# olibridge01/TeXOCR

Measured on AMD Instinct MI355X. Metric: images/sec (OCRModel.generate, greedy, max_len=256, 224x672 px), higher is better.
Workload: dtype bf16; 1 GPU; BASELINE configs[1]: config.yml dims (256-d/8h/4L enc + 4L dec, patch 16, PatchEmbedding C=3), batch 64/GPU, 224x672, greedy max_len=256; global_batch=64, parallelism=dp1 (images sharded, single process, no collective)

## Files before the change

### texocr_amd/csrc/engine.hip

```cpp
#include "../../include/texocr.h"

#include <hip/hip_runtime.h>
#include <hip/hip_ext.h>

#include <algorithm>
#include <array>
#include <cmath>
#include <cstdio>
#include <cstdlib>
#include <chrono>
#include <cstring>
#include <map>
#include <memory>
#include <string>
#include <type_traits>
#include <vector>

namespace txo {
static thread_local std::string g_err;
static int fail(int code, const std::string& msg) { g_err = msg; return code; }
}
#define HIP_TRY(expr)                                                                                   \
    do {                                                                                                \
        hipError_t _e = (expr);                                                                         \
// ... 722 lines not shown
            conv<TB>(s, act[2], b.c2, act[3], B, hc, wc, b.mid, b.mid, 3, b.stride, ri);
            group_norm<true, false>(s, (const TB*)act[3], (const TB*)nullptr, act[3], b.n2, B, ho * wo, b.mid, ro, wo);
            conv<TB>(s, act[3], b.c3, act[2], B, ho, wo, b.mid, b.cout, 1, 1, ro);
            group_norm<true, true>(s, (const TB*)act[2], res, act[0], b.n3, B, ho * wo, b.cout, ro, wo);
            cur = act[0]; hc = ho; wc = wo; mul /= b.stride;
        }
        if (hc != H / 16 || wc != W / 16) return fail(TXO_E_INVALID, "backbone output grid does not match H/16 x W/16");
        *feat = cur;
        HIP_TRY(hipGetLastError());
        return 0;
    }

    int check_image_size(const std::string& who, const char* is, int H, int W, int Hc, int Wc) {
        if (H <= 0 || W <= 0 || H % 16 || W % 16) return fail(TXO_E_INVALID, who + " height/width must be positive multiples of 16");
        if (H > Hc || W > Wc) return fail(TXO_E_INVALID, who + is + "larger than the container");
        if (H > cfg.canvas_h || W > cfg.canvas_w) return fail(TXO_E_INVALID, who + is + "larger than the position-embedding canvas");
        return 0;
    }
    int fixed_batch(int B, int C, int H, int W, ImageBatch* ib) {
        if (!ready) return fail(TXO_E_STATE, "weights not finalized");
        if (C != cfg.in_channels) return fail(TXO_E_INVALID, "image channel count does not match in_channels");
        if (int r = check_image_size("image", " ", H, W, H, W)) return r;
        const int N = 1 + (H / 16) * (W / 16);
        if (B < 1 || B > Bmax) return fail(TXO_E_INVALID, "batch exceeds engine max_batch");
        if (N > Nmax) return fail(TXO_E_INVALID, "token count exceeds engine max_tokens");
        *ib = ImageBatch{B, C, H, W, N};
        return 0;
    }
    int encode(const float* img, int B, int C, int H, int W, float* enc_out, hipStream_t s) override {
        ImageBatch ib;
        if (int r = fixed_batch(B, C, H, W, &ib)) return r;
        return encode_batch(ib, img, enc_out, s);
    }
    int encode_batch(const ImageBatch& ib, const float* img, float* enc_out, hipStream_t s) {
        hipEvent_t e0 = nullptr, e1 = nullptr;
        if (prof) { e0 = pool.next(); e1 = pool.next(); (void)hipEventRecord(e0, s); }
        const int bc = enc_chunk_images(ib.B);
        for (int b0 = 0; b0 < ib.B; b0 += bc) {
            const int nb = std::min(bc, ib.B - b0);
            if (int r = encode_images(ib.chunk(b0, nb), img + b0 * ib.pixels(), enc_out + (size_t)b0 * ib.N * D, s)) return r;
        }
        if (prof) { (void)hipEventRecord(e1, s); ev_enc.push_back({e0, e1}); }
        HIP_TRY(hipGetLastError());
        return 0;
    }
    int enc_chunk_images(int B) const { return knobs.enc_chunk_env > 0 ? std::min(B, knobs.enc_chunk_env) : B; }
    void launch_patch_embed(hipStream_t s, const ImageBatch& ib, const float* img) {
        const int hw = ib.N - 1, w = ib.W / 16, G = cfg.canvas_w / 16;
        const int* rhw = rag_hw + 2 * ib.first;
        auto go = [&](auto load, auto epi) { launch_gemm_big<T>(s, load, patch_w, ib.B * hw, D, ib.C * 256, epi); };
        if (ib.ragged) go(LoadPatchRagged<T>{img, rhw, ib.C, ib.H, ib.W, hw}, EpiPatchRagged{ex, patch_b, pos, rhw, D, hw, G});
        else go(LoadPatch<T>{img, ib.C, ib.H, ib.W, hw, w}, EpiPatch{ex, patch_b, pos, D, hw, w, G});
    }
    const int* ragged_tokens(const ImageBatch& ib) const { return ib.ragged ? rag_ntok + ib.first : nullptr; }
    void launch_enc_attn_f32(hipStream_t s, const ImageBatch& ib, dim3 grid, size_t hs) {
        auto kern = ib.ragged ? enc_attn_kernel<T, true> : enc_attn_kernel<T, false>;
        hipLaunchKernelGGL(kern, grid, dim3(256), 0, s, eqkv, eqkv + hs, eqkv + 2 * hs, eao, ib.N, cfg.enc_heads, ib.B * cfg.enc_heads, ragged_tokens(ib));
    }
    void launch_enc_attn_bf16(hipStream_t s, const ImageBatch& ib, dim3 grid, size_t hs, int rev) {
        const bf16* qb = reinterpret_cast<const bf16*>(eqkv);
        auto kern = ib.ragged ? enc_attn_bf16_v2_kernel<T, true> : enc_attn_bf16_v2_kernel<T, false>;
        hipLaunchKernelGGL(kern, grid, dim3(256), 0, s, qb, qb + hs, qb + 2 * hs, eao, ib.N, cfg.enc_heads, ib.B * cfg.enc_heads, rev, ragged_tokens(ib));
    }
    int encode_images(const ImageBatch& ib, const float* img, float* enc_out, hipStream_t s) {
        const int B = ib.B, H = ib.H, W = ib.W, N = ib.N, hw = N - 1, w = W / 16;
        const int M = B * N, G = cfg.canvas_w / 16;

        hipLaunchKernelGGL(cls_rows_kernel, dim3((B * D + 255) / 256), dim3(256), 0, s, ex, cls, pos, B, N, D);
        if (!hybrid) launch_patch_embed(s, ib, img);
        else if (ib.ragged) {
            const int* rhw = rag_hw + 2 * ib.first;
            const int Hb = rag_box[0], Wb = rag_box[1], hwC = (Hb / 16) * (Wb / 16);
            const size_t n4 = (size_t)M * (D / 4);
            hipLaunchKernelGGL(zero_pad_rows_kernel, dim3((unsigned)((n4 + 255) / 256)), dim3(256), 0, s, ex, ragged_tokens(ib), B, N, D / 4);
            const EpiTokensRagged epi{ex, patch_b, pos, rhw, D, hwC, Wb / 16, N, G};
            if (bk_fp32) {
                const float* feat = nullptr;
                if (int r = backbone<float>(bk32, img, B, Hb, Wb, &feat, s, rhw, H, W)) return r;
                bk_gemm(s, LoadPlain<float>{feat, 1024}, (const float*)bk32.proj_w, B * hwC, D, 1024, epi);
            } else {
                const T* feat = nullptr;
                if (int r = backbone<T>(bk, img, B, Hb, Wb, &feat, s, rhw, H, W)) return r;
                gemm_plain(s, feat, patch_w, B * hwC, D, 1024, epi);
            }
        } else {
            if (bk_fp32) {
                const float* feat = nullptr;
                if (int r = backbone<float>(bk32, img, B, H, W, &feat, s)) return r;
                bk_gemm(s, LoadPlain<float>{feat, 1024}, (const float*)bk32.proj_w, B * hw, D, 1024, EpiTokens{ex, patch_b, pos, D, hw, w, G});
            } else {
                const T* feat = nullptr;
                if (int r = backbone<T>(bk, img, B, H, W, &feat, s)) return r;
                gemm_plain(s, feat, patch_w, B * hw, D, 1024, EpiTokens{ex, patch_b, pos, D, hw, w, G});
            }
        }
        const size_t hs = (size_t)M * Ie;
        bool down = false;
        auto dir = [&]() -> int { if (sizeof(T) != 2) return 0; const bool d = down; down = !down; return d ? 1 : 0; };
        for (int l = 0; l < cfg.enc_layers; ++l) {
            const ResidLN res_x{ey, estats, enc_gb, D}, res_first{ex, nullptr, nullptr, D};
            if (l == 0) launch_ln<0, T>(s, ex, nullptr, ez, enc_g, enc_b, M, dir());
            else launch_ln<3, T>(s, ey, estats, ez, enc_g, enc_b, M, dir());
            const dim3 agrid = ea_grid((N + EA_QBLK - 1) / EA_QBLK, B * cfg.enc_heads);
            if constexpr (sizeof(T) == 4) {
                gemm_plain(s, ez, enc_attn[l].wqkv, M, 3 * Ie, D, EpiHeads<float>{eqkv, hs, Ie, cfg.enc_heads, N});
                launch_enc_attn_f32(s, ib, agrid, hs);
            } else {
                gemm_plain(s, ez, enc_attn[l].wqkv, M, 3 * Ie, D, EpiHeads<bf16>{reinterpret_cast<bf16*>(eqkv), hs, Ie, cfg.enc_heads, N}, dir());
                launch_enc_attn_bf16(s, ib, agrid, hs, dir());
            }
            gemm_plain(s, eao, enc_attn[l].wo, M, 2 * D, Ie,
                               EpiGluRes<sizeof(T) == 2>{ey, l == 0 ? res_first : res_x, enc_attn[l].bo}, dir());
            launch_ln<3, T>(s, ey, estats, ez, enc_g, enc_b, M, dir());
            gemm_plain(s, ez, enc_mlp[l].w1, M, 2 * Fe, D, EpiGeglu<T>{ehid, enc_mlp[l].b1, Fe}, dir());
            gemm_plain(s, ehid, enc_mlp[l].w2, M, D, Fe, EpiBiasRes{ey, res_x, enc_mlp[l].b2}, dir());
        }
        launch_ln<2, float>(s, ey, nullptr, enc_out, encn_g, encn_b, M, dir());
        if (ib.ragged) {
            const size_t n4 = (size_t)M * (D / 4);
            hipLaunchKernelGGL(zero_pad_rows_kernel, dim3((unsigned)((n4 + 255) / 256)), dim3(256), 0, s, enc_out, ragged_tokens(ib), B, N, D / 4);
        }
        return 0;
    }

    int upload_i32(const int32_t* src, int* dst0, int n0, int* dst1, int n1, hipStream_t s) {
        if (rag_ev_pending) { HIP_TRY(hipEventSynchronize(rag_ev)); rag_ev_pending = false; }
        memcpy(rag_host, src, sizeof(int32_t) * (n0 + n1));
        HIP_TRY(hipMemcpyAsync(dst0, rag_host, sizeof(int32_t) * n0, hipMemcpyHostToDevice, s));
        if (n1 > 0) HIP_TRY(hipMemcpyAsync(dst1, rag_host + n0, sizeof(int32_t) * n1, hipMemcpyHostToDevice, s));
        HIP_TRY(hipEventRecord(rag_ev, s));
        rag_ev_pending = true;
        return 0;
    }
    struct Staging { void* dev; const void* host; size_t bytes; };
    template <typename Fill> int ingest_stage(int B, Staging st, hipStream_t s, bool pending, Fill fill) {
        if (B > Bmax) return fail(TXO_E_INVALID, "ingest: batch exceeds engine max_batch (the descriptor staging holds max_batch images)");
        if (ing_ev_pending) { HIP_TRY(hipEventSynchronize(ing_ev)); ing_ev_pending = false; }
        if (int r = fill()) return r;
        HIP_TRY(hipMemcpyAsync(st.dev, st.host, st.bytes, hipMemcpyHostToDevice, s));
        if (pending) { HIP_TRY(hipEventRecord(ing_ev, s)); ing_ev_pending = true; }
        return 0;
    }
    template <typename... P> int ingest_launch(void (*kern)(P...), dim3 grid, dim3 blk, hipStream_t s, typename std::common_type<P>::type... args) {
        if (!prof) { hipLaunchKernelGGL(kern, grid, blk, 0, s, args...); return 0; }
        hipEvent_t e0 = pool.next(), e1 = pool.next();
        if (!e0 || !e1) return fail(TXO_E_HIP, "hipEventCreate failed");
        hipExtLaunchKernelGGL(kern, grid, blk, 0, s, e0, e1, 0, args...);
        ev_ingest.push_back({e0, e1});
        return 0;
    }
// ... 133 lines not shown
    int check_length(int max_len, bool ragged) {
        if (max_len < 1) return fail(TXO_E_INVALID, "max_len must be >= 1");
        if (max_len <= Tmax) return 0;
        if (ragged && !rag_fwd)
            return fail(TXO_E_INVALID, "ragged batches: max_len exceeds the decoder's max_length (the sliding window of a ragged batch needs txo_set_ragged_forward(e, 1))");
        if (V % 8 == 0 && (size_t)Tmax <= (size_t)Bmax * Nmax) return 0;
        return fail(TXO_E_INVALID, ragged ? "ragged batches: max_len exceeds the decoder's max_length and the sliding window's multi-position forward needs a "
                                            "vocabulary size that is a multiple of 8 and max_length <= max_batch * max_tokens"
                                          : "max_len exceeds the decoder's max_length and the sliding window's multi-position forward needs a vocabulary "
                                            "size that is a multiple of 8 and max_length <= max_batch * max_tokens (use decoder.generate's stepwise loop)");
    }
    int check_prefix(const DecodeReq& q, int* m, int* M) {
        const int B = q.src.B, P = q.P;
        if (q.max_len < 1) return fail(TXO_E_INVALID, "prefix decode: max_len must be >= 1");
        if (B < 1 || B > Bmax) return fail(TXO_E_INVALID, "prefix decode: batch exceeds engine max_batch");
        if (P < 1) return fail(TXO_E_INVALID, "prefix decode: the prefix needs at least one column");
        *m = *M = P;
        if (q.prefix_len) {
            *M = 1;
            for (int b = 0; b < B; ++b) {
                if (q.prefix_len[b] < 1 || q.prefix_len[b] > P)
                    return fail(TXO_E_INVALID, "prefix decode: prefix_len[" + std::to_string(b) + "] must be in [1, P]");
                *m = std::min(*m, (int)q.prefix_len[b]); *M = std::max(*M, (int)q.prefix_len[b]);
            }
        }
        if ((long long)*M - 1 + q.max_len > Tmax)
            return fail(TXO_E_INVALID, "prefix decode: the longest prefix - 1 + max_len exceeds the decoder's max_length (a prompted decode does not slide the window)");
        if ((size_t)(*m - 1) > (size_t)Bmax * Nmax)
            return fail(TXO_E_INVALID, "prefix decode: the shortest prefix does not fit the multi-position pass's workspace (max_batch * max_tokens rows)");
        return 0;
    }

    int decode_begin(const float* enc, int B, int N, int eos, hipStream_t s) override { return begin_session(enc, B, N, eos, s, true); }
    int begin_session(const float* enc, int B, int N, int eos, hipStream_t s, bool project_kv, KeyCounts kc = {}, int beams = 1) {
        if (!ready) return fail(TXO_E_STATE, "weights not finalized");
        if (B < 1 || B > Bmax) return fail(TXO_E_INVALID, "batch exceeds engine max_batch");
        if (N < 1 || N > Nmax) return fail(TXO_E_INVALID, "token count exceeds engine max_tokens");
        if (kc.host) { if (int r = upload_i32(kc.host, slens, B, nullptr, 0, s)) return r; }
        if (kc.dev) HIP_TRY(hipMemcpyAsync(slens, kc.dev, sizeof(int) * B, hipMemcpyDeviceToDevice, s));
        {
            const size_t n4 = (size_t)B * N * D / 4;
            hipLaunchKernelGGL((cast_rows_kernel<T>), dim3((n4 + 255) / 256), dim3(256), 0, s, enc, enc_t, n4);
        }
        ses = Session{B * beams, N, B, true, kc.dev || kc.host, project_kv && latent_ok && knobs.lat_mode == 1};
        if (!ses.latent && project_kv) ensure_ckv(s);
        lanes.split(ses.rows, 1, s);
        reset_lanes(s, eos);
        HIP_TRY(hipGetLastError());
        return 0;
    }
    void choose_form(bool row_stop, hipStream_t s) {
        ses.latent = !ses.ragged && latent_ok && (knobs.lat_mode == 1 || (knobs.lat_mode < 0 && auto_latent(ses.rows)));
        ses.row_stop = row_stop;
        ses.lat_self = ses.latent && lat_self_ok() && !row_stop;
        if (!ses.latent) ensure_ckv(s);
    }

    void ensure_ckv(hipStream_t s) {
        if (ses.ckv_valid) return;
        const int M = ses.images * ses.keys;
        gemm_plain(s, enc_t, wckv, M, cfg.dec_layers * 2 * Id, D, EpiHeads<T>{ckv, (size_t)M * Id, Id, cfg.dec_heads, ses.keys});
        ses.ckv_valid = true;
    }

    int abandon_lanes(hipStream_t s, int rc) { stamps.slot = -1; return lanes.abandon(s, ses.images, rc); }
    void reset_lanes(hipStream_t s, int eos, int start_m = 0) {
        for (int i = 0; i < lanes.n; ++i) {
            const LaneSet::Lane& ln = lanes[i];
            const int n = ln.nb > Tmax ? ln.nb : Tmax;
            if (start_m > 0) {
                (void)hipMemsetAsync(st + i, 0, sizeof(StepState), s);
                hipLaunchKernelGGL(prefix_start_kernel, dim3((n + 255) / 256), dim3(256), 0, s, st + i, cur_tok + ln.b0, eos_seen + ln.b0,
                                   done_flag + (size_t)i * Tmax, ln.nb, Tmax, eos, ftab + (size_t)ln.b0 * Tmax, Tmax, flen + ln.b0, start_m);
// ... 559 lines not shown
        }
        if (last_logits) {
            DecGemmArgs<T> f{};
            f.rows = B; f.D = D; f.inner = Id; f.heads = heads; f.tmax = Tmax; f.t_host = t - 1; f.t_ptr = &st[0].t;
            f.N = V; f.K = D; f.W = wlog; f.bias = blog; f.logits = last_logits; f.y = dy; f.gamma = decn_g; f.beta = decn_b;
            if (int r = launch_dec_gemm<PRO_LNF, EPI_LOGITS>(s, f)) return r;
        }
        HIP_TRY(hipGetLastError());
        return 0;
    }

    static constexpr int PERSIST_MAX_BF16_GREEDY = 128;
    bool persist_usable(int B) const {
        if (sample_mode && V > 64 * SR_PER) return false;
        if (prof || prof_cross || g_dbg || knobs.run.stamps || knobs.run.graph >= 0 || knobs.run.lanes > 0) return false;
        if (ses.ragged) return false;
        if (ses.forced) return false;
        if (ses.ruled) return false;
        if (cfg.dec_exp != 4 || cfg.dec_layers > PS_MAXLD) return false;
        const bool exists = (D == 256 && cfg.dec_heads == 8) || (D == 768 && cfg.dec_heads == 12 && sizeof(T) == 2);
        if (!exists) return false;
        if (latent_ok && knobs.lat_mode == 1) return false;
        if (knobs.run.persist >= 0) return knobs.run.persist != 0;
        if (persist_cooldown > 0) return false;
        if (D != 256) return false;
        if (sizeof(T) == 2 && B > PERSIST_MAX_BF16_GREEDY) return false;
        return B <= 256;
    }
    template <int D_, int H_>
    int launch_persist(const PersistArgs<T>& pa, hipStream_t s) {
        const size_t lds = persist_lds_bytes<T, D_, H_>();
        auto kern = pa.logp_out ? (sample_mode ? decode_persist_kernel<T, D_, H_, true, true> : decode_persist_kernel<T, D_, H_, false, true>)
                                : (sample_mode ? decode_persist_kernel<T, D_, H_, true, false> : decode_persist_kernel<T, D_, H_, false, false>);
        if (hipFuncSetAttribute(reinterpret_cast<const void*>(kern), hipFuncAttributeMaxDynamicSharedMemorySize, (int)lds) != hipSuccess) {
            (void)hipGetLastError();
            return fail(TXO_E_STATE, "persistent decode: the device refused the launch's dynamic LDS size");
        }
        if (prof_persist && pool.used + 2 <= pool.ev.size()) {
            hipEvent_t e0 = pool.next(), e1 = pool.next();
            hipExtLaunchKernelGGL(kern, dim3(PS_TEAMS * PS_TEAM_BLOCKS), dim3(PS_THREADS), lds, s, e0, e1, 0, pa);
            ev_persist.push_back({e0, e1});
        } else {
            hipLaunchKernelGGL(kern, dim3(PS_TEAMS * PS_TEAM_BLOCKS), dim3(PS_THREADS), lds, s, pa);
        }
        return 0;
    }
    int generate_persist(const Decode& d, int n_pos, int* n_steps, bool* broke, hipStream_t s) {
        const int B = d.src.B, N = d.src.N, eos = d.q.eos, max_len = n_pos;
        PersistArgs<T> pa{};
        pa.B = B; pa.N = N; pa.V = V; pa.Ld = cfg.dec_layers; pa.Tmax = Tmax; pa.max_len = max_len; pa.eos = eos; pa.bos = cfg.bos;
        for (int l = 0; l < cfg.dec_layers; ++l) {
            PersistLayer<T>& L = pa.L[l];
            L.wqkv = dec_self[l].wqkv; L.wo_s = dec_self[l].wo; L.bo_s = dec_self[l].bo;
            L.wq_c = dec_cross[l].wq; L.wo_c = dec_cross[l].wo; L.bo_c = dec_cross[l].bo;
            L.w1 = dec_mlp[l].w1; L.b1 = dec_mlp[l].b1; L.w2 = dec_mlp[l].w2; L.b2 = dec_mlp[l].b2;
        }
        pa.wlog = wlog;
        {
            bool all = knobs.w_tiled_on && wtiled.count(wlog);
            for (int l = 0; l < cfg.dec_layers && all; ++l)
                all = wtiled.count(dec_self[l].wqkv) && wtiled.count(dec_self[l].wo) && wtiled.count(dec_cross[l].wo) && wtiled.count(dec_mlp[l].w1) && wtiled.count(dec_mlp[l].w2);
            pa.w_tiled = all ? 1 : 0;
            if (all) {
                for (int l = 0; l < cfg.dec_layers; ++l) {
                    PersistLayer<T>& L = pa.L[l];
                    L.wqkv = wtiled.at(dec_self[l].wqkv); L.wo_s = wtiled.at(dec_self[l].wo); L.wo_c = wtiled.at(dec_cross[l].wo);
                    L.w1 = wtiled.at(dec_mlp[l].w1); L.w2 = wtiled.at(dec_mlp[l].w2);
                }
                pa.wlog = wtiled.at(wlog);
// ... 58 lines not shown
            HIP_TRY(hipStreamSynchronize(s));
            HIP_TRY(hipGetLastError());
        }
        return 0;
    }
    int compact_lane(int li, int new_rows, int t1, int eos) {
        auto& ln = lanes[li];
        hipStream_t s = ln.stream;
        const size_t r0 = ln.b0;
        CompactArgs ca{ln.nb, new_rows, (int)r0, cur_tok + r0, eos_seen + r0, row_map + r0, cur_tok2 + r0, row_map2 + r0, cmoves + 2 * r0,
                       cinfo + 2 * li, st + li, eos, ses.ragged ? slens + r0 : nullptr, slens2 + r0};
        hipLaunchKernelGGL(compact_scan_kernel, dim3(1), dim3(1024), 0, s, ca);
        const int heads = cfg.dec_heads;
        auto move = [&](void* base, size_t outer_stride, size_t inner_stride, size_t row_stride, int outer_n, int inner_n, size_t len_elems) {
            MoveArgs ma{reinterpret_cast<unsigned char*>(base), outer_stride * sizeof(T), inner_stride * sizeof(T), row_stride * sizeof(T), inner_n,
                        (unsigned)(len_elems * sizeof(T) / 16), cmoves + 2 * r0, cinfo + 2 * li};
            if (ma.len16 == 0) return;
            hipLaunchKernelGGL(move_rows_kernel, dim3((ma.len16 + 255) / 256, outer_n * inner_n), dim3(256), 0, s, ma);
        };
        move(skv + r0 * heads * Tmax * DH, (size_t)ses.rows * Id * Tmax, (size_t)Tmax * DH, (size_t)heads * Tmax * DH, 2 * cfg.dec_layers, heads, (size_t)t1 * DH);
        if (ses.latent) move(enc_t + r0 * ses.keys * D, 0, 0, (size_t)ses.keys * D, 1, 1, (size_t)ses.keys * D);
        else move(ckv + r0 * ses.keys * Id, (size_t)ses.images * ses.keys * Id, 0, (size_t)ses.keys * Id, 2 * cfg.dec_layers, 1, (size_t)ses.keys * Id);
        ln.nb = new_rows;
        ++last_compactions;
        HIP_TRY(hipGetLastError());
        return 0;
    }
    int generate_impl(const Decode& d, int* steps, hipStream_t s) {
        const DecodeReq& q = d.q;
        const int B = d.src.B, max_len = q.max_len, eos = q.eos;
        const int t0 = d.prompted() ? d.m - 1 : 0;
        const int n_pos = d.prompted() ? d.M + max_len - 1 : std::min(max_len, Tmax);
        const float* rows = d.src.data;
        if (d.src.images) { if (int r = encode_batch(d.src.ib, rows, eenc, s)) return r; rows = eenc; }
        if (int r = begin_session(rows, B, d.src.N, eos, s, false, KeyCounts{d.src.ragged() ? rag_ntok : nullptr})) return r;
        ses.forced = d.prompted();
        ses.ruled = rules_on;
        if (d.prompted()) {
            hipLaunchKernelGGL(prefix_table_kernel, dim3((B * Tmax + 255) / 256), dim3(256), 0, s, ftab, Tmax, q.prefix, q.P, flen, B, V);
            HIP_TRY(hipMemsetAsync(fplogp, 0, sizeof(float) * (size_t)B * Tmax, s));
        }
        last_persist = false;
        if (persist_cooldown > 0) --persist_cooldown;
        if (persist_usable(B)) {
            ensure_ckv(s);
            bool broke = false;
            const int pr = generate_persist(d, n_pos, steps, &broke, s);
            if (pr == 0) {
                last_persist = true; persist_strikes = 0;
                if (!broke && max_len > n_pos) return generate_window(d, n_pos, steps, s);
                return 0;
            }
            if (pr != TXO_E_STATE) return pr;
            ++persist_fallbacks;
            if (++persist_strikes >= 2) {
                persist_cooldown = 64; persist_strikes = 0;
                fprintf(stderr, "[txo] persistent decode launch gave up twice in a row (%s): decoding with launches for the next 64 generates\n", g_err.c_str());
            }
            lanes.split(ses.rows, 1, s);
            reset_lanes(s, eos);
        }
        LoopPlan plan;
        if (int r = plan_loop(d, s, &plan)) return r;
        DonePoll poll{lanes, done_flag, Tmax, n_pos};
        if (int r = run_loop(d, plan, t0, &poll, s)) return r;
        if (int r = deliver(d, plan, poll, steps, s)) return r;
        if (!d.prompted() && !poll.done && max_len > n_pos) return generate_window(d, n_pos, steps, s);
        return 0;
// ... 129 lines not shown
    }

    int beam_refusals(int B, int beams, int max_len) {
        if (beams < 1 || beams > 8) return fail(TXO_E_INVALID, "beams must be in [1, 8]");
        if (max_len < 1 || max_len > Tmax)
            return fail(TXO_E_INVALID, "max_len exceeds the decoder's max_length (a KV cache cannot slide the window)");
        if (Tmax > 1024) return fail(TXO_E_INVALID, "beam search supports max_length <= 1024");
        if (B < 1 || B * beams > Bmax || B * beams > 32767) return fail(TXO_E_INVALID, "images * beams exceeds engine max_batch");
        return 0;
    }
    int beam_search(const DecodeSrc& q, int beams, int max_len, int eos, const BeamSink& sink, int* n_steps, hipStream_t s) override {
        const bool three = sink.best != nullptr;
        if (!three) { last_compactions = 0; last_ragged = false; }
        if (int r = beam_refusals(q.B, beams, max_len)) return r;
        if (!three) {
            if (!sink.out || !sink.out->tokens) return fail(TXO_E_INVALID, "beam search: null out / out->tokens");
            uint32_t ab; memcpy(&ab, &sink.out->length_alpha, sizeof ab);
            const bool nonfinite = (ab & 0x7f800000u) == 0x7f800000u, negative = (ab >> 31) != 0 && (ab << 1) != 0;
            if (nonfinite || negative) return fail(TXO_E_INVALID, "beam search: length_alpha must be finite and >= 0");
        }
        Source src;
        if (int r = resolve_source(q, s, &src)) return r;
        if (!three) last_ragged = src.ragged();
        if (rules_on)
            return fail(TXO_E_INVALID, "beam search: not available while token rules are set (txo_set_token_rules with rules_host == NULL switches them off)");
        const int rc = beam_impl(src, beams, max_len, eos, sink, n_steps, s);
        if (src.ragged()) ses.open = false;
        return rc;
    }
    int beam_impl(const Source& from, int beams, int max_len, int eos, const BeamSink& sink, int* n_steps, hipStream_t s) {
        const int B = from.B, N = from.N, rows = B * beams;
        const ImageBatch* ib = from.batch();
        const float* src = from.data;
        if (ib) { if (int r = encode_batch(*ib, src, eenc, s)) return r; src = eenc; }
        struct Rows { Session& ses; ~Rows() { ses.rows = ses.images; } } restore{ses};
        if (int r = begin_session(src, B, N, eos, s, false, KeyCounts{ib && ib->ragged ? rag_ntok : nullptr}, beams)) return r;
        choose_form(false, s);
        last_persist = false;
        int want = (rows >= 256 && B >= 2 && !prof && !prof_cross && !g_dbg) ? 2 : 1;
        if (knobs.run.lanes > 0) want = std::max(1, std::min(std::min(knobs.run.lanes, MAXL), B));
        if (want == 2 && knobs.tune_lanes && !lanes.tuned) { if (int r = lanes.tune(n_cus, knobs.tune_verbose)) return r; }
        if (want > 1) lanes.split(rows, want, s, beams);
        last_ranges = lanes.n;
        const int n = std::max(rows, Tmax);
        hipLaunchKernelGGL(beam_reset_kernel, dim3((n + 255) / 256), dim3(256), 0, s, st, cur_tok, bscore, bfin, done_flag, rows,
                           beams, Tmax, cfg.bos);
        for (int i = 1; i < lanes.n; ++i)
            hipLaunchKernelGGL(beam_reset_kernel, dim3((Tmax + 255) / 256), dim3(256), 0, s, st + i, cur_tok, bscore, bfin,
                               done_flag + (size_t)i * Tmax, 0, beams, Tmax, cfg.bos);
        if (int r = lanes.fork(s)) return r;
        DonePoll poll{lanes, done_flag, Tmax, max_len};
        const bool want_logp = sink.out && sink.out->logp;
        int cur = 0;
        auto beam_loop = [&]() -> int {
        for (int t = 0; t < max_len; ++t) {
            BeamCtx bm{beams, bpath[cur], bpath[cur ^ 1], want_logp};
            for (int i = 0; i < lanes.n; ++i)
                if (int r2 = enqueue_step(lanes[i].stream, i, nullptr, 0, nullptr, nullptr, eos, &bm, t)) return r2;
            cur ^= 1;
            if (eos < 0) continue;
            if (int r2 = poll.after(t)) return r2;
            if (poll.done) break;
        }
        return 0;
        };
        if (int r = beam_loop()) return abandon_lanes(s, r);
        if (int r = lanes.join(s)) return r;
        const int steps = poll.steps;
        lanes.split(rows, 1, s);
// ... 454 lines not shown
```

### texocr_amd/csrc/gemm_pp.h

```cpp
#pragma once
#include "common.h"
#include "gemm_big.h"

namespace txo {

constexpr int PP_BM = 256, PP_BN = 256, PP_BK = 64, PP_THREADS = 512;
constexpr int PP_TILE_BYTES = PP_BM * 128;
constexpr int PP_BUF_BYTES = 2 * PP_TILE_BYTES;
constexpr int PP_LDS_BYTES = 2 * PP_BUF_BYTES;
constexpr int PP_STAGE_BYTES = 8 * 4096;
constexpr int PP_SMEM_BYTES = PP_LDS_BYTES + PP_STAGE_BYTES;
constexpr int PP_SB_MB = 64;

__device__ inline void dma16(const void* gsrc, unsigned char* lds_base) {
    __builtin_amdgcn_global_load_lds((const __attribute__((address_space(1))) void*)(uintptr_t)gsrc,
                                     (__attribute__((address_space(3))) void*)(uint32_t)(uintptr_t)lds_base, 16, 0, 0);
}

#ifndef PP_SEAM
#define PP_SEAM 1
#endif
#ifdef PP_STAMPS
__device__ unsigned long long g_pp_dbg[4096];
#define PP_STAMP(slot) do { if (blockIdx.x == 0 && lane == 0 && (wave & 3) == 0 && seq < 64) g_pp_dbg[(seq * 2 + wr) * 4 + (slot)] = __builtin_amdgcn_s_memrealtime(); } while (0)
#else
#define PP_STAMP(slot) do {} while (0)
#endif

template <class Epi, bool TR>
__global__ __launch_bounds__(PP_THREADS, 2) void gemm_pp_kernel(const bf16* __restrict__ A, const bf16* __restrict__ W, int M, int N,
                                                                int K, int tiles_n, int n_tiles, int ct, int sbr, int rev, Epi epi) {
    extern __shared__ __attribute__((aligned(1024))) unsigned char lds[];

    const int tid = threadIdx.x, lane = tid & 63;
    const int wave = __builtin_amdgcn_readfirstlane(tid >> 6);
    const int wr = wave >> 2, wc = wave & 3;
    const int lr = lane & 15, lg = lane >> 4;

    const int xcd = blockIdx.x & 7, slot = blockIdx.x >> 3, chunks = gridDim.x >> 3;
    auto tile_seq = [&](int seq) { return (seq * 8 + xcd) * chunks + slot; };
    int n_my = 0;
    while (tile_seq(n_my) < n_tiles) ++n_my;
    if (n_my == 0) return;
    const int tiles_m = n_tiles / tiles_n, sb_tiles = sbr * tiles_n;
    auto tile_origin = [&](int seq, int& m0, int& n0) {
        int L = tile_seq(seq);
        const int sb = L / sb_tiles; L -= sb * sb_tiles;
        const int band_tiles = min(sbr, tiles_m - sb * sbr) * ct;
        const int band = L / band_tiles, k = L - band * band_tiles;
        const int cols = min(ct, tiles_n - band * ct);
        int row = k / cols; const int col = k - row * cols;
        row += sb * sbr;
        if (rev) row = tiles_m - 1 - row;
// ... 126 lines not shown
            if (next_tile) {
                issue_half(0, 0, 1, (g & 1) ^ 1);
                issue_half(0, 1, 1, (g & 1) ^ 1);
            }
        };
        int m0, n0; tile_origin(seq, m0, n0);
        const bool full = m0 + PP_BM <= M;
        relax = next_tile && full;
        if constexpr (TR) {
            __builtin_amdgcn_sched_barrier(0);
            const int strip = n0 + wc * 64;
            int el;
            asm volatile("v_mbcnt_lo_u32_b32 %0, -1, 0\n\tv_mbcnt_hi_u32_b32 %0, -1, %0" : "=v"(el));
            const int elr = el & 15, elg = el >> 4;
            constexpr int NG = Epi::PAIRED ? 1 : 2, NT = NG * 8;
            float cb[NG][32];
            int jout[NG];
#pragma unroll
            for (int c = 0; c < NG; ++c) {
                if constexpr (Epi::PAIRED) {
                    const int nv = strip + (elg >> 1) * 32 + (elg & 1) * 8;
                    epi.cols(nv, nv + 16, cb[c]);
                    jout[c] = (nv >> 5) * 16 + (nv & 15);
                } else {
                    jout[c] = strip + c * 32 + elg * 8;
                    epi.cols(jout[c], cb[c]);
                }
#pragma unroll
                for (int e = 0; e < Epi::NCB; ++e) asm volatile("" : "+v"(cb[c][e]));
            }
            const int mrow = m0 + wr * 128 + elr;
            request_early();
#pragma unroll
            for (int c = 0; c < NG; ++c)
#pragma unroll
                for (int i = 0; i < 8; ++i) {
                    const int m = mrow + i * 16;
                    float rr[10], v[8];
                    if constexpr (Epi::HAS_ROW) epi.rowop(min(m, M - 1), jout[c], rr);
                    if constexpr (Epi::PAIRED) {
                        float gt[8];
#pragma unroll
                        for (int r = 0; r < 4; ++r) { v[r] = acc[i][0][r]; v[4 + r] = acc[i][2][r]; gt[r] = acc[i][1][r]; gt[4 + r] = acc[i][3][r]; }
                        epi.fin(min(m, M - 1), jout[c], v, gt, cb[c], rr, m < M);
                    } else {
#pragma unroll
                        for (int r = 0; r < 4; ++r) { v[r] = acc[i][c * 2][r]; v[4 + r] = acc[i][c * 2 + 1][r]; }
                        epi.fin(min(m, M - 1), jout[c], v, cb[c], rr, m < M);
                    }
                    if constexpr (Epi::HAS_ROW) __builtin_amdgcn_sched_barrier(0);
                }
#pragma unroll
            for (int i = 0; i < 8; ++i)
#pragma unroll
                for (int j = 0; j < 4; ++j) acc[i][j] = f32x4{0.f, 0.f, 0.f, 0.f};
        } else {
            request_early();
            const int nbase = n0 + wc * 64;
            float cb[32];
            int cv, nv;
            if constexpr (Epi::PAIRED) {
                const int vg = lane & 3;
                cv = (vg >> 1) * 32 + (vg & 1) * 8; nv = nbase + cv;
                epi.cols(nv, nv + 16, cb);
            } else {
                cv = (lane & 7) * 8; nv = nbase + cv;
                epi.cols(nv, cb);
            }
            const int jout = Epi::PAIRED ? (nv >> 5) * 16 + (nv & 15) : nv;
            constexpr int ITEMS = Epi::PAIRED ? 1 : 2, RSTEP = Epi::PAIRED ? 16 : 8, RSHIFT = Epi::PAIRED ? 2 : 3;
#pragma unroll
            for (int i = 0; i < 8; ++i) {
                const int mbase = m0 + wr * 128 + i * 16;
                float rr[ITEMS][10];
                if constexpr (Epi::HAS_ROW) {
#pragma unroll
                    for (int q = 0; q < ITEMS; ++q) epi.rowop(min(mbase + (lane >> RSHIFT) + RSTEP * q, M - 1), jout, rr[q]);
                }
#pragma unroll
                for (int j = 0; j < 4; ++j)
#pragma unroll
                    for (int r = 0; r < 4; ++r) stage[sidx(lg * 4 + r, j * 16 + lr)] = acc[i][j][r];
                asm volatile("s_waitcnt lgkmcnt(0)" ::: "memory");
#pragma unroll
// ... 63 lines not shown
```

### texocr_amd/csrc/knobs.h

```cpp
#pragma once
#include "gemm_pp.h"

namespace txo {

inline bool env_set(const char* n) { return getenv(n) != nullptr; }
inline int env_int(const char* n, int unset) { const char* e = getenv(n); return e ? atoi(e) : unset; }
inline int env_bool(const char* n, int unset) { const char* e = getenv(n); return e ? (atoi(e) != 0) : unset; }
inline int env_min1(const char* n, int unset) { const char* e = getenv(n); return e ? std::max(1, atoi(e)) : unset; }
inline bool env_str(const char* n, std::string* v) { const char* e = getenv(n); if (e) *v = e; return e != nullptr; }

static const bool g_dbg = env_set("TXO_DEBUG_SYNC");

struct Knobs {
    struct Run {
        int persist = env_bool("TXO_PERSIST", -1);
        int graph = env_bool("TXO_GRAPH", -1);
        int lanes = env_min1("TXO_LANES", 0);
        std::string stamps_file; bool stamps = env_str("TXO_STAMPS", &stamps_file);
        std::string pstamps_file; bool pstamps = env_str("TXO_PSTAMPS", &pstamps_file);
        bool has_stagger = env_set("TXO_PS_STAGGER_US");
        int stagger_ticks = has_stagger ? (int)(atof(getenv("TXO_PS_STAGGER_US")) * 100.0) : 0;
        bool has_inject = env_set("TXO_PERSIST_INJECT_FAIL");
        int inject_fail = env_int("TXO_PERSIST_INJECT_FAIL", 0);
        void read() { *this = Run{}; }
    } run;
    bool backbone_bf16 = env_set("TXO_BACKBONE_BF16");
    bool bk_exact = env_set("TXO_BACKBONE_EXACT");
    bool self_plain = !env_set("TXO_SELF_FUSED");
    bool dec_wide_off = env_set("TXO_DEC_WIDE_OFF");
    int lat_self_env = env_int("TXO_LATENT_SELF", 0);
    int lat_mode = env_int("TXO_LATENT", -1);
    int lat_g_env = env_int("TXO_LAT_G", 0);
    bool use_pp = !env_set("TXO_GEMM_OLD");
    int pp_tr = env_bool("TXO_PP_TR", -1);
    int pp_ct = env_int("TXO_PP_CT", 0);
    int pp_sb_mb = env_int("TXO_PP_SB_MB", PP_SB_MB);
    int tune_lanes = env_int("TXO_TUNE_LANES", 1);
    bool tune_verbose = env_set("TXO_TUNE_LANES_VERBOSE");
    bool stop_graph_on = env_bool("TXO_STOP_GRAPH", 1);
    int stop_every = env_min1("TXO_STOP_EVERY", 16);
    int stop_gain = env_min1("TXO_STOP_GAIN", 16);
    int enc_chunk_env = env_int("TXO_ENC_CHUNK", -1);
    int w_tiled_on = env_int("TXO_W_TILED", 1);
    int a_tiled_on = env_int("TXO_A_TILED", 1);
    std::string stamps_raw; bool has_stamps_raw = env_str("TXO_STAMPS_RAW", &stamps_raw);
};

}
```

### texocr_amd/csrc/rows.h

```cpp
#pragma once
#include "common.h"

namespace txo {

template <int NV>
__device__ inline void ln_row(float4 (&v)[NV], const float4 (&g)[NV], const float4 (&b)[NV], float inv_d, float* mean_out = nullptr,
                              float* rstd_out = nullptr) {
    float s = 0.f;
#pragma unroll
    for (int i = 0; i < NV; ++i) s += (v[i].x + v[i].y) + (v[i].z + v[i].w);
    const float mean = wave_sum(s) * inv_d;
    float q = 0.f;
#pragma unroll
    for (int i = 0; i < NV; ++i) {
        const float tx = v[i].x - mean, ty = v[i].y - mean, tz = v[i].z - mean, tw = v[i].w - mean;
        q += (tx * tx + ty * ty) + (tz * tz + tw * tw);
    }
    const float rstd = 1.0f / sqrtf(wave_sum(q) * inv_d + LN_EPS);
#pragma unroll
    for (int i = 0; i < NV; ++i) {
        v[i].x = ln_apply(v[i].x, mean, rstd, g[i].x, b[i].x); v[i].y = ln_apply(v[i].y, mean, rstd, g[i].y, b[i].y);
        v[i].z = ln_apply(v[i].z, mean, rstd, g[i].z, b[i].z); v[i].w = ln_apply(v[i].w, mean, rstd, g[i].w, b[i].w);
    }
    if (mean_out) { *mean_out = mean; *rstd_out = rstd; }
// ... 14 lines not shown
                                                      T* __restrict__ z_out, const float* __restrict__ gamma,
                                                      const float* __restrict__ beta, int rows, int rev) {
    const int lane = threadIdx.x & 63;
    int row = blockIdx.x * 4 + (threadIdx.x >> 6);
    if (row >= rows) return;
    if (rev) row = rows - 1 - row;
    constexpr int D = NV * 256;
    const float inv_d = 1.0f / D;
    float4 v[NV], g[NV], b[NV];
#pragma unroll
    for (int i = 0; i < NV; ++i) {
        const int c = i * 256 + lane * 4;
        v[i] = __builtin_bit_cast(float4, MODE == 3 ? ld16_once(in + (size_t)row * D + c) : ld16(in + (size_t)row * D + c));
        g[i] = *reinterpret_cast<const float4*>(gamma + c);
        b[i] = *reinterpret_cast<const float4*>(beta + c);
    }
    if constexpr (MODE == 3) {
        float mean, rstd;
        ln_row<NV>(v, g, b, inv_d, &mean, &rstd);
        if (lane == 0) *reinterpret_cast<float2*>(x_out + (size_t)row * 2) = make_float2(mean, rstd);
        ln_row<NV>(v, g, b, inv_d);
    } else {
        ln_row<NV>(v, g, b, inv_d);
        if constexpr (MODE == 1) {
#pragma unroll
            for (int i = 0; i < NV; ++i) *reinterpret_cast<float4*>(x_out + (size_t)row * D + i * 256 + lane * 4) = v[i];
            ln_row<NV>(v, g, b, inv_d);
        }
    }
#pragma unroll
    for (int i = 0; i < NV; ++i) store4<T>(z_out + (size_t)row * D + i * 256 + lane * 4, v[i]);
}

template <typename T, int MODE>
__global__ __launch_bounds__(256) void ln_rows_generic_kernel(const float* __restrict__ in, float* __restrict__ x_out,
                                                              T* __restrict__ z_out, const float* __restrict__ gamma,
                                                              const float* __restrict__ beta, int rows, int D) {
    const int lane = threadIdx.x & 63;
    const int row = blockIdx.x * 4 + (threadIdx.x >> 6);
    if (row >= rows) return;
    const float inv_d = 1.0f / D;
    const float* src = in + (size_t)row * D;
    if constexpr (MODE == 3) {
        float s = 0.f;
        for (int c = lane; c < D; c += 64) s += src[c];
        const float mean = wave_sum(s) * inv_d;
        float q = 0.f;
        for (int c = lane; c < D; c += 64) { const float d = src[c] - mean; q += d * d; }
        const float rstd = 1.0f / sqrtf(wave_sum(q) * inv_d + LN_EPS);
        if (lane == 0) *reinterpret_cast<float2*>(x_out + (size_t)row * 2) = make_float2(mean, rstd);
        float s2 = 0.f;
        for (int c = lane; c < D; c += 64) s2 += ln_apply(src[c], mean, rstd, gamma[c], beta[c]);
        const float mean2 = wave_sum(s2) * inv_d;
        float q2 = 0.f;
        for (int c = lane; c < D; c += 64) { const float d = ln_apply(src[c], mean, rstd, gamma[c], beta[c]) - mean2; q2 += d * d; }
        const float rstd2 = 1.0f / sqrtf(wave_sum(q2) * inv_d + LN_EPS);
        for (int c = lane; c < D; c += 64)
            z_out[(size_t)row * D + c] = Elem<T>::from_f32(ln_apply(ln_apply(src[c], mean, rstd, gamma[c], beta[c]), mean2, rstd2, gamma[c], beta[c]));
        return;
    }
    for (int pass = 0; pass < (MODE == 1 ? 2 : 1); ++pass) {
        float s = 0.f;
        for (int c = lane; c < D; c += 64) s += src[c];
        const float mean = wave_sum(s) * inv_d;
        float q = 0.f;
        for (int c = lane; c < D; c += 64) { const float d = src[c] - mean; q += d * d; }
// ... 29 lines not shown
```

Measured before the change: 2007 images/sec.

## Fuse final encoder LayerNorm with bf16 cast and cache decode LDS attribute

The final encoder LayerNorm now writes both the fp32 encoder output and the bf16 copy used by the decoder in one pass, and begin_session skips the separate cast_rows_kernel when that copy is already current. This removes one full read and write of the encoder output plus one launch. The persistent-decode dynamic LDS attribute is also set once per device and variant instead of on every launch. A GEMM epilogue loop is reordered to interleave column groups, which changes only instruction scheduling.

```diff
diff --git a/texocr_amd/csrc/engine.hip b/texocr_amd/csrc/engine.hip
--- a/texocr_amd/csrc/engine.hip
+++ b/texocr_amd/csrc/engine.hip
@@ -778,18 +778,22 @@
         if (int r = fixed_batch(B, C, H, W, &ib)) return r;
         return encode_batch(ib, img, enc_out, s);
     }
-    int encode_batch(const ImageBatch& ib, const float* img, float* enc_out, hipStream_t s) {
+    int encode_batch(const ImageBatch& ib, const float* img, float* enc_out, hipStream_t s, bool* enc_t_current = nullptr) {
+        const bool dual = enc_t_current && enc_fused_on() && !ib.ragged && D == 256;
+        if (enc_t_current) *enc_t_current = dual;
         hipEvent_t e0 = nullptr, e1 = nullptr;
         if (prof) { e0 = pool.next(); e1 = pool.next(); (void)hipEventRecord(e0, s); }
         const int bc = enc_chunk_images(ib.B);
         for (int b0 = 0; b0 < ib.B; b0 += bc) {
             const int nb = std::min(bc, ib.B - b0);
-            if (int r = encode_images(ib.chunk(b0, nb), img + b0 * ib.pixels(), enc_out + (size_t)b0 * ib.N * D, s)) return r;
+            const size_t row0 = (size_t)b0 * ib.N * D;
+            if (int r = encode_images(ib.chunk(b0, nb), img + b0 * ib.pixels(), enc_out + row0, s, dual ? enc_t + row0 : nullptr)) return r;
         }
         if (prof) { (void)hipEventRecord(e1, s); ev_enc.push_back({e0, e1}); }
         HIP_TRY(hipGetLastError());
         return 0;
     }
+    bool enc_fused_on() const { return knobs.enc_fused != 0; }
     int enc_chunk_images(int B) const { return knobs.enc_chunk_env > 0 ? std::min(B, knobs.enc_chunk_env) : B; }
     void launch_patch_embed(hipStream_t s, const ImageBatch& ib, const float* img) {
         const int hw = ib.N - 1, w = ib.W / 16, G = cfg.canvas_w / 16;
@@ -808,7 +812,7 @@
         auto kern = ib.ragged ? enc_attn_bf16_v2_kernel<T, true> : enc_attn_bf16_v2_kernel<T, false>;
         hipLaunchKernelGGL(kern, grid, dim3(256), 0, s, qb, qb + hs, qb + 2 * hs, eao, ib.N, cfg.enc_heads, ib.B * cfg.enc_heads, rev, ragged_tokens(ib));
     }
-    int encode_images(const ImageBatch& ib, const float* img, float* enc_out, hipStream_t s) {
+    int encode_images(const ImageBatch& ib, const float* img, float* enc_out, hipStream_t s, T* enc_t_out = nullptr) {
         const int B = ib.B, H = ib.H, W = ib.W, N = ib.N, hw = N - 1, w = W / 16;
         const int M = B * N, G = cfg.canvas_w / 16;
 
@@ -861,7 +865,8 @@
             gemm_plain(s, ez, enc_mlp[l].w1, M, 2 * Fe, D, EpiGeglu<T>{ehid, enc_mlp[l].b1, Fe}, dir());
             gemm_plain(s, ehid, enc_mlp[l].w2, M, D, Fe, EpiBiasRes{ey, res_x, enc_mlp[l].b2}, dir());
         }
-        launch_ln<2, float>(s, ey, nullptr, enc_out, encn_g, encn_b, M, dir());
+        if (enc_t_out) hipLaunchKernelGGL((ln_final_dual_kernel<T, 1>), dim3((M + 3) / 4), dim3(256), 0, s, ey, enc_out, enc_t_out, encn_g, encn_b, M, dir());
+        else launch_ln<2, float>(s, ey, nullptr, enc_out, encn_g, encn_b, M, dir());
         if (ib.ragged) {
             const size_t n4 = (size_t)M * (D / 4);
             hipLaunchKernelGGL(zero_pad_rows_kernel, dim3((unsigned)((n4 + 255) / 256)), dim3(256), 0, s, enc_out, ragged_tokens(ib), B, N, D / 4);
@@ -1061,13 +1066,13 @@
     }
 
     int decode_begin(const float* enc, int B, int N, int eos, hipStream_t s) override { return begin_session(enc, B, N, eos, s, true); }
-    int begin_session(const float* enc, int B, int N, int eos, hipStream_t s, bool project_kv, KeyCounts kc = {}, int beams = 1) {
+    int begin_session(const float* enc, int B, int N, int eos, hipStream_t s, bool project_kv, KeyCounts kc = {}, int beams = 1, bool enc_t_current = false) {
         if (!ready) return fail(TXO_E_STATE, "weights not finalized");
         if (B < 1 || B > Bmax) return fail(TXO_E_INVALID, "batch exceeds engine max_batch");
         if (N < 1 || N > Nmax) return fail(TXO_E_INVALID, "token count exceeds engine max_tokens");
         if (kc.host) { if (int r = upload_i32(kc.host, slens, B, nullptr, 0, s)) return r; }
         if (kc.dev) HIP_TRY(hipMemcpyAsync(slens, kc.dev, sizeof(int) * B, hipMemcpyDeviceToDevice, s));
-        {
+        if (!enc_t_current) {
             const size_t n4 = (size_t)B * N * D / 4;
             hipLaunchKernelGGL((cast_rows_kernel<T>), dim3((n4 + 255) / 256), dim3(256), 0, s, enc, enc_t, n4);
         }
@@ -1693,9 +1698,16 @@
         const size_t lds = persist_lds_bytes<T, D_, H_>();
         auto kern = pa.logp_out ? (sample_mode ? decode_persist_kernel<T, D_, H_, true, true> : decode_persist_kernel<T, D_, H_, false, true>)
                                 : (sample_mode ? decode_persist_kernel<T, D_, H_, true, false> : decode_persist_kernel<T, D_, H_, false, false>);
-        if (hipFuncSetAttribute(reinterpret_cast<const void*>(kern), hipFuncAttributeMaxDynamicSharedMemorySize, (int)lds) != hipSuccess) {
-            (void)hipGetLastError();
-            return fail(TXO_E_STATE, "persistent decode: the device refused the launch's dynamic LDS size");
+        static bool attr_set[64][4] = {};
+        int dev = 0;
+        (void)hipGetDevice(&dev);
+        bool* const have = (enc_fused_on() && dev >= 0 && dev < 64) ? &attr_set[dev][(pa.logp_out ? 2 : 0) + (sample_mode ? 1 : 0)] : nullptr;
+        if (!have || !*have) {
+            if (hipFuncSetAttribute(reinterpret_cast<const void*>(kern), hipFuncAttributeMaxDynamicSharedMemorySize, (int)lds) != hipSuccess) {
+                (void)hipGetLastError();
+                return fail(TXO_E_STATE, "persistent decode: the device refused the launch's dynamic LDS size");
+            }
+            if (have) *have = true;
         }
         if (prof_persist && pool.used + 2 <= pool.ev.size()) {
             hipEvent_t e0 = pool.next(), e1 = pool.next();
@@ -1820,8 +1832,9 @@
         const int t0 = d.prompted() ? d.m - 1 : 0;
         const int n_pos = d.prompted() ? d.M + max_len - 1 : std::min(max_len, Tmax);
         const float* rows = d.src.data;
-        if (d.src.images) { if (int r = encode_batch(d.src.ib, rows, eenc, s)) return r; rows = eenc; }
-        if (int r = begin_session(rows, B, d.src.N, eos, s, false, KeyCounts{d.src.ragged() ? rag_ntok : nullptr})) return r;
+        bool enc_t_current = false;
+        if (d.src.images) { if (int r = encode_batch(d.src.ib, rows, eenc, s, &enc_t_current)) return r; rows = eenc; }
+        if (int r = begin_session(rows, B, d.src.N, eos, s, false, KeyCounts{d.src.ragged() ? rag_ntok : nullptr}, 1, enc_t_current)) return r;
         ses.forced = d.prompted();
         ses.ruled = rules_on;
         if (d.prompted()) {
@@ -2017,9 +2030,10 @@
         const int B = from.B, N = from.N, rows = B * beams;
         const ImageBatch* ib = from.batch();
         const float* src = from.data;
-        if (ib) { if (int r = encode_batch(*ib, src, eenc, s)) return r; src = eenc; }
+        bool enc_t_current = false;
+        if (ib) { if (int r = encode_batch(*ib, src, eenc, s, &enc_t_current)) return r; src = eenc; }
         struct Rows { Session& ses; ~Rows() { ses.rows = ses.images; } } restore{ses};
-        if (int r = begin_session(src, B, N, eos, s, false, KeyCounts{ib && ib->ragged ? rag_ntok : nullptr}, beams)) return r;
+        if (int r = begin_session(src, B, N, eos, s, false, KeyCounts{ib && ib->ragged ? rag_ntok : nullptr}, beams, enc_t_current)) return r;
         choose_form(false, s);
         last_persist = false;
         int want = (rows >= 256 && B >= 2 && !prof && !prof_cross && !g_dbg) ? 2 : 1;
diff --git a/texocr_amd/csrc/gemm_pp.h b/texocr_amd/csrc/gemm_pp.h
--- a/texocr_amd/csrc/gemm_pp.h
+++ b/texocr_amd/csrc/gemm_pp.h
@@ -19,6 +19,9 @@
 
 #ifndef PP_SEAM
 #define PP_SEAM 1
+#endif
+#ifndef PP_HALVES_ADJ
+#define PP_HALVES_ADJ 1
 #endif
 #ifdef PP_STAMPS
 __device__ unsigned long long g_pp_dbg[4096];
@@ -211,9 +214,9 @@
             const int mrow = m0 + wr * 128 + elr;
             request_early();
 #pragma unroll
-            for (int c = 0; c < NG; ++c)
-#pragma unroll
-                for (int i = 0; i < 8; ++i) {
+            for (int it = 0; it < NG * 8; ++it) {
+                {
+                    const int c = PP_HALVES_ADJ ? it % NG : it / 8, i = PP_HALVES_ADJ ? it / NG : it % 8;
                     const int m = mrow + i * 16;
                     float rr[10], v[8];
                     if constexpr (Epi::HAS_ROW) epi.rowop(min(m, M - 1), jout[c], rr);
@@ -229,6 +232,7 @@
                     }
                     if constexpr (Epi::HAS_ROW) __builtin_amdgcn_sched_barrier(0);
                 }
+            }
 #pragma unroll
             for (int i = 0; i < 8; ++i)
 #pragma unroll
diff --git a/texocr_amd/csrc/knobs.h b/texocr_amd/csrc/knobs.h
--- a/texocr_amd/csrc/knobs.h
+++ b/texocr_amd/csrc/knobs.h
@@ -40,6 +40,7 @@
     bool stop_graph_on = env_bool("TXO_STOP_GRAPH", 1);
     int stop_every = env_min1("TXO_STOP_EVERY", 16);
     int stop_gain = env_min1("TXO_STOP_GAIN", 16);
+    int enc_fused = env_int("TXO_ENC_FUSED", 1);
     int enc_chunk_env = env_int("TXO_ENC_CHUNK", -1);
     int w_tiled_on = env_int("TXO_W_TILED", 1);
     int a_tiled_on = env_int("TXO_A_TILED", 1);
diff --git a/texocr_amd/csrc/rows.h b/texocr_amd/csrc/rows.h
--- a/texocr_amd/csrc/rows.h
+++ b/texocr_amd/csrc/rows.h
@@ -70,6 +70,30 @@
     for (int i = 0; i < NV; ++i) store4<T>(z_out + (size_t)row * D + i * 256 + lane * 4, v[i]);
 }
 
+template <typename T, int NV>
+__global__ __launch_bounds__(256) void ln_final_dual_kernel(const float* __restrict__ in, float* __restrict__ z_out, T* __restrict__ t_out,
+                                                            const float* __restrict__ gamma, const float* __restrict__ beta, int rows, int rev) {
+    const int lane = threadIdx.x & 63;
+    int row = blockIdx.x * 4 + (threadIdx.x >> 6);
+    if (row >= rows) return;
+    if (rev) row = rows - 1 - row;
+    constexpr int D = NV * 256;
+    float4 v[NV], g[NV], b[NV];
+#pragma unroll
+    for (int i = 0; i < NV; ++i) {
+        const int c = i * 256 + lane * 4;
+        v[i] = __builtin_bit_cast(float4, ld16(in + (size_t)row * D + c));
+        g[i] = *reinterpret_cast<const float4*>(gamma + c);
+        b[i] = *reinterpret_cast<const float4*>(beta + c);
+    }
+    ln_row<NV>(v, g, b, 1.0f / D);
+#pragma unroll
+    for (int i = 0; i < NV; ++i) {
+        store4<float>(z_out + (size_t)row * D + i * 256 + lane * 4, v[i]);
+        store4<T>(t_out + (size_t)row * D + i * 256 + lane * 4, v[i]);
+    }
+}
+
 template <typename T, int MODE>
 __global__ __launch_bounds__(256) void ln_rows_generic_kernel(const float* __restrict__ in, float* __restrict__ x_out,
                                                               T* __restrict__ z_out, const float* __restrict__ gamma,
```

Result: no change. 1994 images/sec (-0.7%).
